# zaki699/Real-Time-Video-Quality-Analysis

Hardware: AMD Instinct MI355X
Metric: frames/sec (higher is better)
Workload: dtype u8->f32 (SSE/bins/SAD exact int); 1 GPU; 1920x1080 full suite (motion-SAD, DCT, temporal-DCT, Canny, ORB count, gray+colour hist) + PSNR/SSIM; id=c3, streams=1, inflight=2, collective=none, rehearsal_single_device=False, resident=HBM, ssim_mode=gauss, pixfmt=bgr24, dct_mode=block8, motion=sad, parallelism=1 stream/GPU x1, overlap=True, launched_by=direct

## Files before the change

### real-time-video-quality-analysis_amd/csrc/k_gray_hist.hip

```cpp
#include "vqa_dev.hpp"
#include "vqa_kernels.hpp"
#include "vqa_math.hpp"

namespace vqa {

enum { F_GRAY_HIST = 1, F_COLOR_HIST = 2, F_SUM2 = 4 };

__device__ __forceinline__ uint32_t byte_of(const uint32_t *d, int k) { return (d[k >> 2] >> ((k & 3) * 8)) & 0xffu; }

template <bool VEC>
__global__ __launch_bounds__(256) void k_bgr2gray_hist(const uint8_t *__restrict__ bgr, int h, int w,
                                                       int64_t frame_stride, int64_t row_stride,
                                                       uint8_t *__restrict__ gray, int gp, int64_t plane_stride,
                                                       vqa_frame_metrics *__restrict__ res, uint32_t flags)
{
    __shared__ uint32_t lh[4 * 256 * 8];
    __shared__ unsigned long long red[4];
    const int f = blockIdx.y;
    const bool hg = (flags & F_GRAY_HIST) && res, hc = (flags & F_COLOR_HIST) && res;
    const bool any_hist = hg || hc;
    if (any_hist) {
        for (int i = threadIdx.x; i < 4 * 256 * 8; i += 256) lh[i] = 0;
        __syncthreads();
    }
    const unsigned cp = threadIdx.x & 7u;
    const uint8_t *src = bgr + (int64_t)f * frame_stride;
    uint8_t *dst = gray + (int64_t)f * plane_stride;
    const int cpr = (w + 15) >> 4;
    const int total = h * cpr;
    unsigned long long s2 = 0;
    for (int c = blockIdx.x * 256 + threadIdx.x; c < total; c += gridDim.x * 256) {
        const int y = c / cpr;
        const int x0 = (c - y * cpr) << 4;
        const uint8_t *p = src + (int64_t)y * row_stride + (int64_t)x0 * 3;
        uint32_t d[12];
        int npx = 16;
        if (VEC) {
            const uint4 v0 = ((const uint4 *)p)[0], v1 = ((const uint4 *)p)[1], v2 = ((const uint4 *)p)[2];
            d[0] = v0.x; d[1] = v0.y; d[2] = v0.z; d[3] = v0.w;
            d[4] = v1.x; d[5] = v1.y; d[6] = v1.z; d[7] = v1.w;
            d[8] = v2.x; d[9] = v2.y; d[10] = v2.z; d[11] = v2.w;
        } else {
            npx = min(16, w - x0);
#pragma unroll
            for (int k = 0; k < 12; k++) d[k] = 0;
            for (int k = 0; k < npx * 3; k++) d[k >> 2] |= (uint32_t)p[k] << ((k & 3) * 8);
        }
        uint32_t g[16];
        uint32_t sq = 0;
#pragma unroll
        for (int i = 0; i < 16; i++) {
            const uint32_t b = byte_of(d, 3 * i), gg = byte_of(d, 3 * i + 1), r = byte_of(d, 3 * i + 2);
            g[i] = bgr2gray_u8(b, gg, r);
            if (VEC || i < npx) {
                sq += g[i] * g[i];
                if (hg) atomicAdd(&lh[(g[i] << 3) | cp], 1u);
                if (hc) {
                    atomicAdd(&lh[((256u + b) << 3) | cp], 1u);
                    atomicAdd(&lh[((512u + gg) << 3) | cp], 1u);
                    atomicAdd(&lh[((768u + r) << 3) | cp], 1u);
                }
            }
        }
        s2 += sq;
        uint8_t *q = dst + (int64_t)y * gp + x0;
        if (VEC) {
            uint4 o;
            o.x = g[0] | (g[1] << 8) | (g[2] << 16) | (g[3] << 24);
            o.y = g[4] | (g[5] << 8) | (g[6] << 16) | (g[7] << 24);
            o.z = g[8] | (g[9] << 8) | (g[10] << 16) | (g[11] << 24);
            o.w = g[12] | (g[13] << 8) | (g[14] << 16) | (g[15] << 24);
            *(uint4 *)q = o;
        } else {
            for (int i = 0; i < npx; i++) q[i] = (uint8_t)g[i];
        }
    }
    if (!res) return;
    if (any_hist) {
        __syncthreads();
        for (int i = threadIdx.x; i < 4 * 256; i += 256) {
            const uint4 c0 = *(const uint4 *)&lh[i * 8], c1 = *(const uint4 *)&lh[i * 8 + 4];
            const uint32_t v = c0.x + c0.y + c0.z + c0.w + c1.x + c1.y + c1.z + c1.w;
            if (v) {
                const int which = i >> 8, bin = i & 255;
                uint32_t *gdst = which == 0 ? &res[f].hist_gray[bin] : &res[f].hist_bgr[which - 1][bin];
                atomicAdd(gdst, v);
            }
        }
    }
    if (flags & F_SUM2) {
        const unsigned long long t = block_sum_u64(s2, red);
        if (threadIdx.x == 0 && t) atomicAdd((unsigned long long *)&res[f].sum_gray2, t);
    }
}

__global__ __launch_bounds__(256) void k_resize_planes(const uint8_t *__restrict__ bgr, int h, int w,
                                                       int64_t frame_stride, int64_t row_stride, int rw, int rh,
                                                       const int32_t *__restrict__ xofs, const int32_t *__restrict__ xa,
                                                       const int32_t *__restrict__ yofs, const int32_t *__restrict__ yb,
                                                       int mode, uint8_t *__restrict__ planeA,
                                                       uint8_t *__restrict__ planeB, int pp, int64_t plane_stride,
                                                       vqa_frame_metrics *__restrict__ res, uint32_t flags)
{
    __shared__ uint32_t lh[4][256];
    __shared__ unsigned long long red[4];
    const int f = blockIdx.y;
    const bool hg = (flags & F_GRAY_HIST) && res, hc = (flags & F_COLOR_HIST) && res;
    if (hg || hc) {
        for (int i = threadIdx.x; i < 4 * 256; i += 256) (&lh[0][0])[i] = 0;
        __syncthreads();
    }
    const int idx = blockIdx.x * 256 + threadIdx.x;
    unsigned long long s2 = 0;
    if (idx < rw * rh) {
        const int oy = idx / rw, ox = idx - oy * rw;
        int sx0, sx1, sy0, sy1, a0, a1, b0, b1;
        if (mode == 1) {
            sx0 = 2 * ox; sx1 = sx0 + 1; sy0 = 2 * oy; sy1 = sy0 + 1;
            a0 = a1 = b0 = b1 = 0;
        } else {
            sx0 = xofs[ox]; sx1 = min(sx0 + 1, w - 1);
            a0 = xa[2 * ox]; a1 = xa[2 * ox + 1];
            const int sy = yofs[oy];
            sy0 = min(max(sy, 0), h - 1); sy1 = min(max(sy + 1, 0), h - 1);
            b0 = yb[2 * oy]; b1 = yb[2 * oy + 1];
        }
        const uint8_t *src = bgr + (int64_t)f * frame_stride;
        const uint8_t *p00 = src + (int64_t)sy0 * row_stride + (int64_t)sx0 * 3;
        const uint8_t *p01 = src + (int64_t)sy0 * row_stride + (int64_t)sx1 * 3;
        const uint8_t *p10 = src + (int64_t)sy1 * row_stride + (int64_t)sx0 * 3;
        const uint8_t *p11 = src + (int64_t)sy1 * row_stride + (int64_t)sx1 * 3;
        uint32_t c00[3], c01[3], c10[3], c11[3];
#pragma unroll
        for (int k = 0; k < 3; k++) { c00[k] = p00[k]; c01[k] = p01[k]; c10[k] = p10[k]; c11[k] = p11[k]; }
        const uint32_t g00 = bgr2gray_u8(c00[0], c00[1], c00[2]), g01 = bgr2gray_u8(c01[0], c01[1], c01[2]);
        const uint32_t g10 = bgr2gray_u8(c10[0], c10[1], c10[2]), g11 = bgr2gray_u8(c11[0], c11[1], c11[2]);
        uint32_t ga, rc[3];
        if (mode == 1) {
            ga = (g00 + g01 + g10 + g11 + 2) >> 2;
#pragma unroll
            for (int k = 0; k < 3; k++) rc[k] = (c00[k] + c01[k] + c10[k] + c11[k] + 2) >> 2;
        } else {
            ga = resize_vcombine((int)(g00 * a0 + g01 * a1), (int)(g10 * a0 + g11 * a1), b0, b1);
#pragma unroll
            for (int k = 0; k < 3; k++)
                rc[k] = resize_vcombine((int)(c00[k] * a0 + c01[k] * a1), (int)(c10[k] * a0 + c11[k] * a1), b0, b1);
        }
        const uint32_t gb = bgr2gray_u8(rc[0], rc[1], rc[2]);
        planeA[(int64_t)f * plane_stride + (int64_t)oy * pp + ox] = (uint8_t)ga;
        if (planeB) planeB[(int64_t)f * plane_stride + (int64_t)oy * pp + ox] = (uint8_t)gb;
        s2 = (unsigned long long)(ga * ga);
        if (hg) atomicAdd(&lh[0][gb], 1u);
        if (hc) { atomicAdd(&lh[1][rc[0]], 1u); atomicAdd(&lh[2][rc[1]], 1u); atomicAdd(&lh[3][rc[2]], 1u); }
    }
    if (!res) return;
    if (hg || hc) {
        __syncthreads();
        for (int i = threadIdx.x; i < 4 * 256; i += 256) {
            const uint32_t v = (&lh[0][0])[i];
            if (v) {
                const int which = i >> 8, bin = i & 255;
                atomicAdd(which == 0 ? &res[f].hist_gray[bin] : &res[f].hist_bgr[which - 1][bin], v);
            }
        }
    }
    if (flags & F_SUM2) {
        const unsigned long long t = block_sum_u64(s2, red);
        if (threadIdx.x == 0 && t) atomicAdd((unsigned long long *)&res[f].sum_gray2, t);
    }
}


void launch_bgr2gray_hist(hipStream_t st, const uint8_t *bgr, int n, int h, int w, int64_t frame_stride,
                          int64_t row_stride, uint8_t *gray, int gp, int64_t plane_stride, vqa_frame_metrics *res,
                          bool gray_hist, bool color_hist, bool sum2)
{
    if (n <= 0) return;
    const uint32_t flags = (gray_hist ? F_GRAY_HIST : 0) | (color_hist ? F_COLOR_HIST : 0) | (sum2 ? F_SUM2 : 0);
    const bool vec = (w % 16 == 0) && (((uintptr_t)bgr | (uintptr_t)gray) % 16 == 0) && (frame_stride % 16 == 0) &&
                     (row_stride % 16 == 0) && (gp % 16 == 0) && (plane_stride % 16 == 0);
    const int chunks = h * ((w + 15) / 16);
    int bpf = (chunks + 256 * 8 - 1) / (256 * 8);
    bpf = bpf < 1 ? 1 : (bpf > 256 ? 256 : bpf);
    dim3 grid(bpf, n), block(256);
    if (vec)
        hipLaunchKernelGGL(k_bgr2gray_hist<true>, grid, block, 0, st, bgr, h, w, frame_stride, row_stride, gray, gp,
                           plane_stride, res, flags);
    else
        hipLaunchKernelGGL(k_bgr2gray_hist<false>, grid, block, 0, st, bgr, h, w, frame_stride, row_stride, gray, gp,
                           plane_stride, res, flags);
}

void launch_resize_planes(hipStream_t st, const uint8_t *bgr, int n, int h, int w, int64_t frame_stride,
                          int64_t row_stride, int rw, int rh, const int32_t *xofs, const int32_t *xa,
                          const int32_t *yofs, const int32_t *yb, int mode, uint8_t *planeA, uint8_t *planeB, int pp,
                          int64_t plane_stride, vqa_frame_metrics *res, bool gray_hist, bool color_hist, bool sum2)
{
    if (n <= 0) return;
    const uint32_t flags = (gray_hist ? F_GRAY_HIST : 0) | (color_hist ? F_COLOR_HIST : 0) | (sum2 ? F_SUM2 : 0);
    dim3 grid((rw * rh + 255) / 256, n), block(256);
    hipLaunchKernelGGL(k_resize_planes, grid, block, 0, st, bgr, h, w, frame_stride, row_stride, rw, rh, xofs, xa, yofs,
                       yb, mode, planeA, planeB, pp, plane_stride, res, flags);
}

}
```

### real-time-video-quality-analysis_amd/csrc/vqa_capi.hip

```cpp
#include <hip/hip_runtime.h>

#include <cmath>
#include <cstddef>
#include <cstdio>
#include <cstdlib>
#include <cstring>
#include <map>
#include <string>
#include <tuple>
#include <vector>

#include "vqa_kernels.hpp"

using namespace vqa;

namespace {

struct dbuf {
    void *p = nullptr;
    size_t cap = 0;
};

struct hbuf {
    void *p = nullptr;
// ... 656 lines not shown

void vqa_default_params(vqa_params *p)
{
    if (!p) return;
    memset(p, 0, sizeof *p);
    p->canny_low = 100;
    p->canny_high = 200;
    p->sad_range = 7;
    p->dct_mode = VQA_DCT_AUTO;
}

int vqa_create(int device, vqa_ctx **out)
{
    if (!out) return VQA_ERR_INVALID;
    *out = nullptr;
    int n = 0;
    if (hipGetDeviceCount(&n) != hipSuccess || n <= 0) return VQA_ERR_NO_DEVICE;
    if (device < 0 || device >= n) return VQA_ERR_NO_DEVICE;
    vqa_ctx *c = new (std::nothrow) vqa_ctx();
    if (!c) return VQA_ERR_OOM;
    c->device = device;
    if (hipSetDevice(device) != hipSuccess || hipStreamCreateWithFlags(&c->stream, hipStreamNonBlocking) != hipSuccess) {
        delete c;
        return VQA_ERR_HIP;
    }
    c->dct_wave_slots = dct8_wave_slots();
    if (const char *e = getenv("VQA_OVERLAP")) c->opt_overlap = atoi(e) != 0;
#ifdef VQA_TEST_SEAMS
    if (const char *e = getenv("VQA_HYST_MAX_ROUNDS")) c->seam_hyst_max_rounds = atoi(e) > 0 ? atoi(e) : 0;
    if (const char *e = getenv("VQA_HYST_RESCUE_MAX_ROUNDS")) c->seam_hyst_rescue_max_rounds = atoi(e) > 0 ? atoi(e) : 0;
    if (const char *e = getenv("VQA_FAIL_ENSURE_AT")) c->seam_fail_at = atol(e);
    if (const char *e = getenv("VQA_FB_CHUNK_BYTES")) c->seam_fb_chunk_bytes = atoll(e);
#endif
    *out = c;
    return VQA_OK;
}

int vqa_set_option(vqa_ctx *c, int option, int value)
{
    if (!c) return VQA_ERR_INVALID;
    if (busy(c)) return VQA_ERR_STATE;
    switch (option) {
    case VQA_OPT_OVERLAP: c->opt_overlap = value != 0; return VQA_OK;
    case VQA_OPT_HYST_STATS: c->opt_hyst_stats = value != 0; return VQA_OK;
    default: return VQA_ERR_INVALID;
    }
}

int vqa_get_option(const vqa_ctx *c, int option, int *value)
{
    if (!c || !value) return VQA_ERR_INVALID;
    switch (option) {
    case VQA_OPT_OVERLAP: *value = c->opt_overlap ? 1 : 0; return VQA_OK;
    case VQA_OPT_HYST_STATS: *value = c->opt_hyst_stats ? 1 : 0; return VQA_OK;
    default: return VQA_ERR_INVALID;
    }
}

int vqa_build_flavour(void)
{
    int f = 0;
#ifdef VQA_AB_VARIANTS
    f |= 1;
#endif
#ifdef VQA_TEST_SEAMS
    f |= 2;
#endif
    return f;
}

static void release_scratch(vqa_ctx *c)
{
    dbuf *bufs[] = {&c->gray_full, &c->planeA, &c->planeB, &c->state, &c->res_dev, &c->partials, &c->tile_flags,
                    &c->dirty0, &c->dirty1, &c->again_dev, &c->stage_frames, &c->stage_prev, &c->dct_scratch,
                    &c->dct_pe, &c->dct_pt, &c->qres_dev, &c->qpartials, &c->qstage_ref, &c->qstage_dist,
                    &c->qms_pyr, &c->qms_dev, &c->vif_pyr, &c->vif_acc, &c->vif_dev, &c->adm_pyr, &c->adm_part, &c->adm_sums, &c->mot_acc, &c->mot_stage, &c->mot_prev, &c->fb_tmp, &c->fb_blur, &c->fb_img, &c->fb_R, &c->fb_M, &c->fb_flow0, &c->fb_flow1, &c->fb_part};
    for (dbuf *b : bufs) release(*b);
    for (auto &kv : c->tabs) free_table(kv.second.v);
    for (auto &kv : c->fb_tabs) free_table(kv.second.v);
    for (auto &kv : c->dct_mats) free_table(kv.second.v);
    for (auto &kv : c->fft_plans) free_table(kv.second.v);
    c->tabs.clear(); c->fb_tabs.clear(); c->dct_mats.clear(); c->fft_plans.clear();
    for (hbuf *b : {&c->res_host, &c->qres_host, &c->qms_host, &c->vif_host, &c->adm_host, &c->mot_host}) {
        if (b->p) (void)hipHostFree(b->p);
        b->p = nullptr; b->cap = 0;
    }
    c->last_n = 0; c->last_has_full = c->last_has_state = c->last_has_planes = false;
}

int vqa_trim(vqa_ctx *c)
{
    if (!c) return VQA_ERR_INVALID;
    if (busy(c)) return VQA_ERR_STATE;
    HIPCHK(c, hipSetDevice(c->device));
    if (int rc = sync_all(c)) return rc;
    prof_collect(c);
    release_scratch(c);
    (void)hipGetLastError();
    return VQA_OK;
}

int vqa_destroy(vqa_ctx *c)
{
    if (!c) return VQA_ERR_INVALID;
    (void)hipSetDevice(c->device);
    (void)sync_all(c);
    release_scratch(c);
    for (auto &t : c->ev_open) { (void)hipEventDestroy(std::get<1>(t)); (void)hipEventDestroy(std::get<2>(t)); }
    for (hipEvent_t e : c->ev_pool) (void)hipEventDestroy(e);
    for (int i = 0; i < 3; i++) {
        if (c->side[i]) (void)hipStreamDestroy(c->side[i]);
        if (c->ev_join[i]) (void)hipEventDestroy(c->ev_join[i]);
    }
    if (c->ev_fork) (void)hipEventDestroy(c->ev_fork);
    if (c->ev_xctx) (void)hipEventDestroy(c->ev_xctx);
    for (int i = 0; i < 6; i++)
        if (c->fb_ev[i]) (void)hipEventDestroy(c->fb_ev[i]);
    (void)hipStreamDestroy(c->stream);
    delete c;
    return VQA_OK;
}

const char *vqa_last_hip_error(const vqa_ctx *c) { return c ? c->last_err.c_str() : ""; }

int vqa_alloc_pinned(vqa_ctx *c, size_t bytes, void **out)
{
    if (!c || !out || !bytes) return VQA_ERR_INVALID;
    HIPCHK(c, hipSetDevice(c->device));
    HIPCHK(c, hipHostMalloc(out, bytes, hipHostMallocDefault));
    return VQA_OK;
}
int vqa_free_pinned(vqa_ctx *c, void *p)
{
    if (!c || !p) return VQA_ERR_INVALID;
    HIPCHK(c, hipHostFree(p));
    return VQA_OK;
}
static bool host_byte_is_pinned(const void *p)
{
    hipPointerAttribute_t a;
    memset(&a, 0, sizeof a);
    if (hipPointerGetAttributes(&a, p) != hipSuccess) {
        (void)hipGetLastError();
        return false;
    }
    return a.type == hipMemoryTypeHost;
}
int vqa_host_is_pinned(vqa_ctx *c, const void *p, size_t bytes, int *out)
{
    if (!c || !p || !out || !bytes) return VQA_ERR_INVALID;
    *out = (host_byte_is_pinned(p) && host_byte_is_pinned((const uint8_t *)p + (bytes - 1))) ? 1 : 0;
    return VQA_OK;
}
int vqa_alloc_device(vqa_ctx *c, size_t bytes, void **out)
{
    if (!c || !out || !bytes) return VQA_ERR_INVALID;
    HIPCHK(c, hipSetDevice(c->device));
    HIPCHK(c, hipMalloc(out, bytes));
    return VQA_OK;
}
int vqa_free_device(vqa_ctx *c, void *p)
{
    if (!c || !p) return VQA_ERR_INVALID;
    HIPCHK(c, hipFree(p));
    return VQA_OK;
}
int vqa_copy_h2d(vqa_ctx *c, void *dst, const void *src, size_t bytes)
{
    if (!c || !dst || !src) return VQA_ERR_INVALID;
    HIPCHK(c, hipSetDevice(c->device));
    HIPCHK(c, hipMemcpyAsync(dst, src, bytes, hipMemcpyHostToDevice, c->stream));
    return VQA_OK;
}
int vqa_stream_wait(vqa_ctx *waiter, vqa_ctx *signaler)
{
    if (!waiter || !signaler || waiter == signaler) return VQA_ERR_INVALID;
    if (waiter->device != signaler->device) return VQA_ERR_INVALID;
    HIPCHK(waiter, hipSetDevice(waiter->device));
    if (!signaler->ev_xctx) HIPCHK(waiter, hipEventCreateWithFlags(&signaler->ev_xctx, hipEventDisableTiming));
    HIPCHK(waiter, hipEventRecord(signaler->ev_xctx, signaler->stream));
    HIPCHK(waiter, hipStreamWaitEvent(waiter->stream, signaler->ev_xctx, 0));
    return VQA_OK;
}
int vqa_copy_d2h(vqa_ctx *c, void *dst, const void *src, size_t bytes)
{
    if (!c || !dst || !src) return VQA_ERR_INVALID;
    HIPCHK(c, hipSetDevice(c->device));
    HIPCHK(c, hipMemcpyAsync(dst, src, bytes, hipMemcpyDeviceToHost, c->stream));
    return VQA_OK;
}
int vqa_sync(vqa_ctx *c)
{
    if (!c) return VQA_ERR_INVALID;
    return sync_all(c);
}
void *vqa_stream(vqa_ctx *c) { return c ? (void *)c->stream : nullptr; }
extern "C" __attribute__((visibility("hidden"))) int vqa_ctx_device_(const vqa_ctx *c) { return c->device; }
extern "C" __attribute__((visibility("hidden"))) void *vqa_ctx_stream_(const vqa_ctx *c) { return (void *)c->stream; }

static int drain_failed_submit(vqa_ctx *c, int rc, bool touched)
{
    if (rc != VQA_OK && touched) {
        const std::string why = c->last_err;
        (void)sync_all(c);
        (void)hipGetLastError();
        prof_discard(c);
        c->last_err = why;
    }
    return rc;
}

static int complexity_submit_body(vqa_ctx *c, const uint8_t *frames, const uint8_t *prev0, int mem_kind, int n, int h, int w,
                                  int64_t frame_stride, int64_t row_stride, uint32_t mask, const vqa_params *params,
                                  bool &touched)
{
    if (!c || !frames || n <= 0 || h <= 0 || w <= 0) return VQA_ERR_INVALID;
    if (mem_kind != VQA_MEM_HOST && mem_kind != VQA_MEM_DEVICE) return VQA_ERR_INVALID;
    if (!mask || (mask & ~VQA_M_ALL)) return VQA_ERR_INVALID;
    if (row_stride < (int64_t)3 * w || frame_stride < row_stride * (h - 1) + (int64_t)3 * w) return VQA_ERR_INVALID;
    if (c->pend_c) return VQA_ERR_STATE;
    vqa_params P;
    if (params) P = *params; else vqa_default_params(&P);
    for (int i = 0; i < 9; i++)
        if (P.reserved[i]) return VQA_ERR_INVALID;
    if (P.motion_mode != VQA_MOTION_SAD && P.motion_mode != VQA_MOTION_FARNEBACK) return VQA_ERR_INVALID;
    if (P.sad_range < 0 || P.sad_range > 7) return VQA_ERR_INVALID;
    if (P.resize_w < 0 || P.resize_h < 0 || ((P.resize_w == 0) != (P.resize_h == 0))) return VQA_ERR_INVALID;
    if (P.dct_mode < VQA_DCT_AUTO || P.dct_mode > VQA_DCT_FULL) return VQA_ERR_INVALID;
    if ((int64_t)h * w > (1ll << 28)) return VQA_ERR_UNSUPPORTED;
    HIPCHK(c, hipSetDevice(c->device));
    hipStream_t st = c->stream;
    touched = true;

    const int rw = P.resize_w ? P.resize_w : w, rh = P.resize_h ? P.resize_h : h;
    const bool resized = !(rw == w && rh == h);
    const int ph = rh, pw = rw;
    const int pp = align_up(pw, 64), gp = align_up(w, 64);
    const bool want_gh = mask & VQA_M_GRAY_HIST, want_ch = mask & VQA_M_COLOR_HIST, want_dct = mask & VQA_M_DCT;
    const bool want_t = mask & VQA_M_TEMPORAL_DCT, want_e = mask & VQA_M_EDGE, want_m = mask & VQA_M_MOTION;
    const bool want_orb = mask & VQA_M_ORB;
    const bool batch_has_prev0 = prev0 != nullptr;

    const uint8_t *dframes = frames, *dprev = prev0;
    if (mem_kind == VQA_MEM_HOST) {
        const size_t rbytes = (size_t)3 * w, fbytes = rbytes * h;
        const bool padded = (size_t)row_stride != rbytes;
        int rc = ensure(c, c->stage_frames, fbytes * n);
        if (rc) return rc;
        if (!padded && (size_t)frame_stride == fbytes) {
            HIPCHK(c, hipMemcpyAsync(c->stage_frames.p, frames, fbytes * n, hipMemcpyHostToDevice, st));
        } else {
            for (int i = 0; i < n; i++) {
                uint8_t *dst = (uint8_t *)c->stage_frames.p + fbytes * i;
                const uint8_t *src = frames + (int64_t)i * frame_stride;
                if (padded)
                    HIPCHK(c, hipMemcpy2DAsync(dst, rbytes, src, (size_t)row_stride, rbytes, h, hipMemcpyHostToDevice, st));
                else
                    HIPCHK(c, hipMemcpyAsync(dst, src, fbytes, hipMemcpyHostToDevice, st));
            }
        }
        dframes = (const uint8_t *)c->stage_frames.p;
        if (batch_has_prev0) {
            rc = ensure(c, c->stage_prev, fbytes);
            if (rc) return rc;
            if (padded)
                HIPCHK(c, hipMemcpy2DAsync(c->stage_prev.p, rbytes, prev0, (size_t)row_stride, rbytes, h,
                                           hipMemcpyHostToDevice, st));
            else
                HIPCHK(c, hipMemcpyAsync(c->stage_prev.p, prev0, fbytes, hipMemcpyHostToDevice, st));
            dprev = (const uint8_t *)c->stage_prev.p;
        }
        frame_stride = (int64_t)fbytes;
        row_stride = (int64_t)rbytes;
    }

    int rc = ensure(c, c->res_dev, sizeof(vqa_frame_metrics) * (size_t)n);
    if (rc) return rc;
    rc = ensure_pinned(c, c->res_host, sizeof(vqa_frame_metrics) * (size_t)n);
    if (rc) return rc;
    HIPCHK(c, hipMemsetAsync(c->res_dev.p, 0, sizeof(vqa_frame_metrics) * (size_t)n, st));
    vqa_frame_metrics *const res_all = (vqa_frame_metrics *)c->res_dev.p;
    const uint8_t *const dframes_all = dframes, *const dprev_all = dprev;
    const int n_all = n;

    const int SLICE = 32768;
    auto run_slice = [&](const int a0) -> int {
    const int n = n_all - a0 < SLICE ? n_all - a0 : SLICE;
    const uint8_t *dframes = dframes_all + (int64_t)a0 * frame_stride;
    const uint8_t *dprev = a0 ? dframes_all + (int64_t)(a0 - 1) * frame_stride : dprev_all;
    const bool has_prev0 = a0 > 0 || batch_has_prev0;
    vqa_frame_metrics *res = res_all + a0;

    const bool want_plane = want_gh || want_ch || want_dct || want_t || want_e;
    const bool need_full = (!resized && want_plane) || want_m;
    const bool need_planes = resized && want_plane;
    const int64_t full_stride = (int64_t)h * gp, plane_stride = (int64_t)ph * pp;
    uint8_t *gfull = nullptr, *pA = nullptr, *pB = nullptr;
    if (need_full) {
        rc = ensure(c, c->gray_full, (size_t)full_stride * (n + 1));
        if (rc) return rc;
        gfull = (uint8_t *)c->gray_full.p;
        const bool prev_needed = has_prev0 && (want_m || (!resized && want_t));
        prof_scope ps_(c, VQA_K_GRAY_HIST);
        if (prev_needed)
            launch_bgr2gray_hist(st, dprev, 1, h, w, frame_stride, row_stride, gfull, gp, full_stride, nullptr, false,
                                 false, false);
        launch_bgr2gray_hist(st, dframes, n, h, w, frame_stride, row_stride, gfull + full_stride, gp, full_stride, res,
                             !resized && want_gh, !resized && want_ch, !resized && want_dct);
    }
    if (need_planes) {
        resize_tabs T;
        rc = get_tabs(c, h, w, rh, rw, T);
        if (rc) return rc;
        rc = ensure(c, c->planeA, (size_t)plane_stride * (n + 1));
        if (rc) return rc;
        rc = ensure(c, c->planeB, (size_t)plane_stride * n);
        if (rc) return rc;
        pA = (uint8_t *)c->planeA.p;
        pB = (uint8_t *)c->planeB.p;
        prof_scope ps_(c, VQA_K_RESIZE);
        if (has_prev0 && want_t)
            launch_resize_planes(st, dprev, 1, h, w, frame_stride, row_stride, rw, rh, T.xofs, T.xa, T.yofs, T.yb,
                                 T.mode, pA, nullptr, pp, plane_stride, nullptr, false, false, false);
        launch_resize_planes(st, dframes, n, h, w, frame_stride, row_stride, rw, rh, T.xofs, T.xa, T.yofs, T.yb, T.mode,
                             pA + plane_stride, pB, pp, plane_stride, res, want_gh, want_ch, want_dct);
    } else if (!resized) {
        pA = gfull;
        pB = gfull + full_stride;
    }

    int dct_mode_eff = P.dct_mode;
    if (dct_mode_eff == VQA_DCT_AUTO) dct_mode_eff = ((int64_t)ph * pw <= 128 * 128) ? VQA_DCT_FULL : VQA_DCT_BLOCK8;
    const bool use_side[3] = {c->opt_overlap && want_m && P.motion_mode == VQA_MOTION_SAD, c->opt_overlap && want_e,
                              c->opt_overlap && (want_dct || want_t) && dct_mode_eff == VQA_DCT_FULL && (want_m || want_e)};
    const bool overlap = use_side[0] || use_side[1] || use_side[2];
    hipStream_t st_sad = st, st_canny = st, st_dct = st;
    if (overlap) {
        for (int i = 0; i < 3; i++) {
            if (!use_side[i]) continue;
            if (!c->side[i]) HIPCHK(c, hipStreamCreateWithFlags(&c->side[i], hipStreamNonBlocking));
            if (!c->ev_join[i]) HIPCHK(c, hipEventCreateWithFlags(&c->ev_join[i], hipEventDisableTiming));
        }
        if (!c->ev_fork) HIPCHK(c, hipEventCreateWithFlags(&c->ev_fork, hipEventDisableTiming));
        HIPCHK(c, hipEventRecord(c->ev_fork, st));
        if (use_side[0]) { st_sad = c->side[0]; HIPCHK(c, hipStreamWaitEvent(st_sad, c->ev_fork, 0)); }
        if (use_side[1]) { st_canny = c->side[1]; HIPCHK(c, hipStreamWaitEvent(st_canny, c->ev_fork, 0)); }
        if (use_side[2]) { st_dct = c->side[2]; HIPCHK(c, hipStreamWaitEvent(st_dct, c->ev_fork, 0)); }
    }

    if (want_dct || want_t) {
        const int mode = dct_mode_eff;
        if (mode == VQA_DCT_BLOCK8) {
            const int pb = dct8_blocks_per_frame(ph, pw);
            rc = ensure(c, c->partials, sizeof(double) * 2 * (size_t)pb * n);
            if (rc) return rc;
            prof_scope ps_(c, VQA_K_DCT8);
            launch_dct8(st, pA, pp, plane_stride, n, ph, pw, want_dct, want_t, has_prev0, (double *)c->partials.p, res, c->dct_wave_slots);
        } else {
            if (dct_fft_supported(ph, pw)) {
                dct_fft_plan Pw, Ph;
                rc = get_fft_plan(c, pw, &Pw);
                if (rc) return rc;
                rc = get_fft_plan(c, ph, &Ph);
                if (rc) return rc;
                const size_t tiles = (size_t)dct_fft_tiles(ph, pw);
                rc = ensure(c, c->dct_scratch, sizeof(float) * 2 * (size_t)ph * pw * n);
                if (rc) return rc;
                rc = ensure(c, c->dct_pe, sizeof(double) * tiles * n);
                if (rc) return rc;
                rc = ensure(c, c->dct_pt, sizeof(double) * tiles * n);
                if (rc) return rc;
                prof_scope ps_(c, VQA_K_DCT_FULL, st_dct);
                launch_dct_full_fft(st_dct, pA, pp, plane_stride, n, ph, pw, Pw, Ph, (float *)c->dct_scratch.p, (double *)c->dct_pe.p,
                                    (double *)c->dct_pt.p, want_dct, want_t, has_prev0, res);
            } else {
                float *cw = nullptr, *ch = nullptr;
                rc = get_dct_matrix(c, pw, &cw);
                if (rc) return rc;
                rc = get_dct_matrix(c, ph, &ch);
                if (rc) return rc;
                const size_t tiles = (size_t)((ph + 15) / 16) * ((pw + 15) / 16);
                rc = ensure(c, c->dct_scratch, sizeof(float) * (size_t)ph * pw * n);
                if (rc) return rc;
                rc = ensure(c, c->dct_pe, sizeof(double) * tiles * n);
                if (rc) return rc;
                rc = ensure(c, c->dct_pt, sizeof(double) * tiles * n);
                if (rc) return rc;
                prof_scope ps_(c, VQA_K_DCT_FULL, st_dct);
                launch_dct_full(st_dct, pA, pp, plane_stride, n, ph, pw, cw, ch, (float *)c->dct_scratch.p,
                                (double *)c->dct_pe.p, (double *)c->dct_pt.p, want_dct, want_t, has_prev0, res);
            }
        }
    }

    if (want_m && P.motion_mode == VQA_MOTION_SAD) {
        prof_scope ps_(c, VQA_K_SAD, st_sad);
        launch_block_sad(st_sad, gfull, gp, full_stride, n, h, w, P.sad_range, has_prev0, res);
    } else if (want_m) {
        prof_scope ps_(c, VQA_K_FARNEBACK);
        rc = run_farneback(c, st, gfull, gp, full_stride, n, h, w, has_prev0, res);
        if (rc) return rc;
    }

    c->last_has_state = false;
    if (want_e) {
        const int ww = (pw + 63) / 64;
        const size_t words = (size_t)n * ((ph + 63) / 64) * ww * 64;
        const unsigned ntiles = canny_hyst_tiles(n, ph, pw);
        rc = ensure(c, c->state, sizeof(uint64_t) * words * 2);
        if (rc) return rc;
        rc = ensure(c, c->tile_flags, sizeof(uint32_t) * ntiles * 2);
        if (rc) return rc;
        const size_t NS = CANNY_HYST_SEGMENTS;
        rc = ensure(c, c->dirty0, sizeof(uint32_t) * ntiles * NS);
        if (rc) return rc;
        rc = ensure(c, c->dirty1, sizeof(uint32_t) * ntiles * NS);
        if (rc) return rc;
        rc = ensure(c, c->again_dev, sizeof(uint32_t) * 3 * n * NS);
        if (rc) return rc;
        unsigned long long *strong = (unsigned long long *)c->state.p, *weak = strong + words;
        unsigned *queued[2] = {(unsigned *)c->tile_flags.p, (unsigned *)c->tile_flags.p + ntiles};
        unsigned *lists[2] = {(unsigned *)c->dirty0.p, (unsigned *)c->dirty1.p};
        unsigned *counts = (unsigned *)c->again_dev.p;
        HIPCHK(c, hipMemsetAsync(queued[0], 0, sizeof(uint32_t) * ntiles * 2, st_canny));
        HIPCHK(c, hipMemsetAsync(counts, 0, sizeof(uint32_t) * 3 * n * NS, st_canny));
        auto cnt = [&](int r) { return counts + (size_t)(r % 3) * n * NS; };
        int lo = P.canny_low, hi = P.canny_high;
        if (lo > hi) { int t = lo; lo = hi; hi = t; }
        {
            prof_scope ps_(c, VQA_K_CANNY_NMS, st_canny);
            launch_canny_nms(st_canny, pB, pp, plane_stride, n, ph, pw, lo, hi, strong, weak, res);
        }
        int round = 0;
        {
            prof_scope ps_(c, VQA_K_CANNY_HYST, st_canny);
            launch_canny_hyst_all(st_canny, strong, weak, n, ph, pw, queued[1], lists[1], cnt(1), res, c->opt_hyst_stats);
        }
        {
            prof_scope ps_(c, VQA_K_CANNY_HYST, st_canny);
            const canny_geom cg = canny_tiles(ph, pw);
            int WIDE = (cg.tiles_x * cg.tiles_y > 1024 && n < 256) ? 8 : 6;
#ifdef VQA_AB_VARIANTS
            { static const int e = ab_knob("VQA_HYST_WIDE", 0); if (e > 0) WIDE = e; }
#endif
            for (round = 1; round <= WIDE; round++) {
                const int in = round & 1, out = in ^ 1;
#ifdef VQA_AB_VARIANTS
                static const bool trace = ab_knob("VQA_HYST_TRACE", 0) != 0;
                if (trace) {
                    std::vector<uint32_t> hc((size_t)n * NS);
                    (void)hipStreamSynchronize(st_canny);
                    (void)hipMemcpy(hc.data(), cnt(round), sizeof(uint32_t) * hc.size(), hipMemcpyDeviceToHost);
                    unsigned long long tot = 0;
                    for (uint32_t v : hc) tot += v;
                    fprintf(stderr, "[hyst] round %d: %llu of %u tiles queued\n", round, tot, ntiles);
                }
#endif
                launch_canny_hyst_list(st_canny, strong, weak, n, ph, pw, queued[in], lists[in], cnt(round), queued[out], lists[out],
                                       cnt(round + 1), cnt(round + 2), res, c->opt_hyst_stats);
            }
            unsigned *tc[2];
            tc[round & 1] = cnt(round);
            tc[(round & 1) ^ 1] = cnt(round + 1);
            launch_canny_hyst_tail(st_canny, strong, weak, n, ph, pw, lists[0], tc[0], queued[0], lists[1], tc[1], queued[1],
                                   round & 1, res, c->opt_hyst_stats, c->seam_hyst_max_rounds, c->seam_hyst_rescue_max_rounds);
        }
        launch_canny_finish(st_canny, strong, n, ph, pw, res);
        c->last_has_state = true;
    }

    if (want_orb) {
        resize_tabs T64;
        rc = get_tabs(c, h, w, 64, 64, T64);
        if (rc) return rc;
        prof_scope ps_(c, VQA_K_ORB);
        launch_orb64(st, dframes, n, h, w, frame_stride, row_stride, T64.xofs, T64.xa, T64.yofs, T64.yb, T64.mode, res);
    }
    if (overlap) {
        hipStream_t ss[3] = {st_sad, st_canny, st_dct};
        for (int i = 0; i < 3; i++) {
            if (!use_side[i]) continue;
            HIPCHK(c, hipEventRecord(c->ev_join[i], ss[i]));
            HIPCHK(c, hipStreamWaitEvent(st, c->ev_join[i], 0));
        }
    }
    c->last_n = n; c->last_has_full = need_full; c->last_has_planes = need_planes;
    return VQA_OK;
    };
    for (int a0 = 0; a0 < n_all; a0 += SLICE)
        if (const int src = run_slice(a0)) return src;
    const bool has_prev0 = batch_has_prev0;

    HIPCHK(c, hipGetLastError());
    if (want_gh || want_ch) {
        HIPCHK(c, hipMemcpyAsync(c->res_host.p, c->res_dev.p, sizeof(vqa_frame_metrics) * (size_t)n, hipMemcpyDeviceToHost, st));
        c->pend_c_tail_only = false;
    } else {
        const size_t off = offsetof(vqa_frame_metrics, sum_gray2), tail = sizeof(vqa_frame_metrics) - off;
        HIPCHK(c, hipMemcpy2DAsync((uint8_t *)c->res_host.p + off, sizeof(vqa_frame_metrics), (uint8_t *)c->res_dev.p + off,
                                   sizeof(vqa_frame_metrics), tail, (size_t)n, hipMemcpyDeviceToHost, st));
        c->pend_c_tail_only = true;
    }
    c->pend_c = n;
    c->pend_c_prev0 = has_prev0;
    c->last_h = h; c->last_w = w; c->last_ph = ph; c->last_pw = pw; c->last_pp = pp; c->last_gp = gp;
    c->last_resized = resized;
    return VQA_OK;
}

int vqa_complexity_submit(vqa_ctx *c, const uint8_t *frames, const uint8_t *prev0, int mem_kind, int n, int h, int w,
                          int64_t frame_stride, int64_t row_stride, uint32_t mask, const vqa_params *params)
{
    bool touched = false;
    const int rc = complexity_submit_body(c, frames, prev0, mem_kind, n, h, w, frame_stride, row_stride, mask, params, touched);
    return drain_failed_submit(c, rc, touched);
}

int vqa_complexity_wait(vqa_ctx *c, vqa_frame_metrics *out, int n)
{
    if (!c || !out) return VQA_ERR_INVALID;
    if (!c->pend_c || n != c->pend_c) return VQA_ERR_STATE;
    HIPCHK(c, hipStreamSynchronize(c->stream));
    prof_collect(c);
    memcpy(out, c->res_host.p, sizeof(vqa_frame_metrics) * (size_t)n);
    for (int i = 0; i < n; i++) {
        if (c->pend_c_tail_only) memset(&out[i], 0, offsetof(vqa_frame_metrics, sum_gray2));
        out[i].has_prev = (i > 0 || c->pend_c_prev0) ? 1u : 0u;
    }
    c->pend_c = 0;
    for (int i = 0; i < n; i++)
        if (out[i].hyst_overflow == 1u) {
            c->last_err = "Canny hysteresis of frame " + std::to_string(i) + " of " + std::to_string(n) +
                          " stopped before its fixpoint (edge_count " + std::to_string(out[i].edge_count) +
                          " would be a lower bound): records withheld";
            memset(out, 0, sizeof(vqa_frame_metrics) * (size_t)n);
            return VQA_ERR_INCOMPLETE;
        }
    return VQA_OK;
}

extern "C++" {

static bool bad_batch_args(const vqa_ctx *c, const void *ref, const void *dist, int mem_kind, int n, const vqa_plane_desc *planes,
                           int n_planes)
{
    return !c || !ref || !dist || n <= 0 || !planes || n_planes <= 0 || n_planes > 4 ||
           (mem_kind != VQA_MEM_HOST && mem_kind != VQA_MEM_DEVICE);
}

struct plane_batch {
    int depth, bps;
    int64_t span;
};

template <class F> static int check_planes(const vqa_plane_desc *planes, int n_planes, plane_batch &B, F limits)
{
    B.depth = planes[0].bit_depth == 0 ? 8 : planes[0].bit_depth;
    if (B.depth < 8 || B.depth > 16) return VQA_ERR_INVALID;
    B.bps = B.depth > 8 ? 2 : 1;
    B.span = 0;
    for (int p = 0; p < n_planes; p++) {
        const vqa_plane_desc &d = planes[p];
        if ((d.bit_depth == 0 ? 8 : d.bit_depth) != B.depth) return VQA_ERR_INVALID;
        if (B.bps == 2 && ((d.offset | d.row_stride | (int64_t)d.pixel_step) & 1)) return VQA_ERR_INVALID;
        if (d.width <= 0 || d.height <= 0 || d.offset < 0 || d.pixel_step <= 0 ||
            d.row_stride < (int64_t)d.width * d.pixel_step - (d.pixel_step - B.bps))
            return VQA_ERR_INVALID;
        if (int rc = limits(d)) return rc;
        const int64_t end = d.offset + (int64_t)(d.height - 1) * d.row_stride + (int64_t)(d.width - 1) * d.pixel_step + B.bps;
        B.span = end > B.span ? end : B.span;
    }
    return VQA_OK;
}

static int side_and_area_limits(const vqa_plane_desc &d, int min_dim)
{
    if (d.width < min_dim || d.height < min_dim) return VQA_ERR_UNSUPPORTED;
    if ((int64_t)d.width * d.height > (1ll << 28)) return VQA_ERR_UNSUPPORTED;
    return VQA_OK;
}

static int stage(vqa_ctx *c, dbuf &buf, const uint8_t *&frames, size_t bytes)
{
    if (int rc = ensure(c, buf, bytes)) return rc;
    HIPCHK(c, hipMemcpyAsync(buf.p, frames, bytes, hipMemcpyHostToDevice, c->stream));
    frames = (const uint8_t *)buf.p;
    return VQA_OK;
}

static int stage_pair(vqa_ctx *c, int mem_kind, int n, int64_t span, const uint8_t *&ref, int64_t ref_fs, const uint8_t *&dist,
                      int64_t dist_fs)
{
    if (mem_kind != VQA_MEM_HOST) return VQA_OK;
    if (int rc = stage(c, c->qstage_ref, ref, (size_t)(n - 1) * ref_fs + span)) return rc;
    return stage(c, c->qstage_dist, dist, (size_t)(n - 1) * dist_fs + span);
}

constexpr int QSLICE = 32768;

template <class F> static void for_each_slice(int n, F body)
{
    for (int a0 = 0; a0 < n; a0 += QSLICE) body(a0, n - a0 < QSLICE ? n - a0 : QSLICE);
}

template <class F> static void for_each_group(const vqa_plane_desc *planes, int n_planes, F body)
{
    bool done[4] = {false, false, false, false};
    for (int p = 0; p < n_planes; p++) {
        if (done[p]) continue;
        int idx[4], cnt = 0;
        for (int q = p; q < n_planes; q++) {
// ... 412 lines not shown
```

### real-time-video-quality-analysis_amd/csrc/vqa_kernels.hpp

```cpp
#pragma once
#include <hip/hip_runtime.h>
#include <stdint.h>

#include "../../include/vqa.h"

#ifdef VQA_AB_VARIANTS
#include <cstdlib>
#endif

namespace vqa {

inline int ab_knob(const char *name, int dflt)
{
#ifdef VQA_AB_VARIANTS
    const char *e = getenv(name);
    return e ? atoi(e) : dflt;
#else
    (void)name;
    return dflt;
#endif
}

void launch_bgr2gray_hist(hipStream_t st, const uint8_t *bgr, int n, int h, int w, int64_t frame_stride,
                          int64_t row_stride, uint8_t *gray, int gp, int64_t plane_stride, vqa_frame_metrics *res,
                          bool gray_hist, bool color_hist, bool sum2);
void launch_resize_planes(hipStream_t st, const uint8_t *bgr, int n, int h, int w, int64_t frame_stride,
                          int64_t row_stride, int rw, int rh, const int32_t *xofs, const int32_t *xa,
                          const int32_t *yofs, const int32_t *yb, int mode, uint8_t *planeA, uint8_t *planeB, int pp,
                          int64_t plane_stride, vqa_frame_metrics *res, bool gray_hist, bool color_hist, bool sum2);

void launch_orb64(hipStream_t st, const uint8_t *bgr, int n, int h, int w, int64_t frame_stride, int64_t row_stride,
                  const int32_t *xofs, const int32_t *xa, const int32_t *yofs, const int32_t *yb, int mode,
                  vqa_frame_metrics *res);

int dct8_blocks_per_frame(int h, int w);
int dct8_wave_slots();
void launch_dct8(hipStream_t st, const uint8_t *planes, int pitch, int64_t plane_stride, int n, int h, int w,
                 bool energy, bool temporal, bool first_has_prev, double *partials, vqa_frame_metrics *res, int wave_slots);

void launch_dct_full(hipStream_t st, const uint8_t *planes, int pitch, int64_t plane_stride, int n, int h, int w,
                     const float *cw, const float *ch, float *scratch, double *pe, double *pt, bool energy,
                     bool temporal, bool first_has_prev, vqa_frame_metrics *res);

void launch_dct_full_finalize(hipStream_t st, const double *pe, const double *pt, int tiles, int n, vqa_frame_metrics *res,
                              bool energy, bool temporal, bool first_has_prev);

constexpr int DCT_FFT_MAX_PASSES = 12;
struct dct_fft_plan {
    int n, npass;
    int radix[DCT_FFT_MAX_PASSES];
    int m[DCT_FFT_MAX_PASSES], tstep[DCT_FFT_MAX_PASSES];
    uint32_t ns_magic[DCT_FFT_MAX_PASSES];
    const float2 *tw;
    const float2 *post;
};
bool dct_fft_factor(int n, int radix[DCT_FFT_MAX_PASSES], int *npass);
bool dct_fft_supported(int h, int w);
int dct_fft_tiles(int h, int w);
void launch_dct_full_fft(hipStream_t st, const uint8_t *planes, int pitch, int64_t plane_stride, int n, int h, int w,
                         const dct_fft_plan &plan_w, const dct_fft_plan &plan_h, float *scratch, double *pe, double *pt,
                         bool energy, bool temporal, bool first_has_prev, vqa_frame_metrics *res);

struct canny_geom {
    int tiles_x, tiles_y;
};
canny_geom canny_tiles(int h, int w);
void launch_canny_nms(hipStream_t st, const uint8_t *gray, int pitch, int64_t plane_stride, int n, int h, int w,
                      int low, int high, unsigned long long *strong, unsigned long long *weak,
                      vqa_frame_metrics *res);
unsigned canny_hyst_tiles(int n, int h, int w);
constexpr int CANNY_HYST_SEGMENTS = 16;
void launch_canny_hyst_all(hipStream_t st, unsigned long long *strong, const unsigned long long *weak, int n, int h,
                           int w, unsigned *queued, unsigned *out_list, unsigned *out_count, vqa_frame_metrics *res,
                           int stats);
void launch_canny_hyst_list(hipStream_t st, unsigned long long *strong, const unsigned long long *weak, int n, int h,
                            int w, unsigned *in_queued, const unsigned *in_list, const unsigned *in_count,
                            unsigned *out_queued, unsigned *out_list, unsigned *out_count, unsigned *zero_count,
                            vqa_frame_metrics *res, int stats);
void launch_canny_hyst_tail(hipStream_t st, unsigned long long *strong, const unsigned long long *weak, int n, int h,
                            int w, unsigned *list0, unsigned *cnt0, unsigned *q0, unsigned *list1, unsigned *cnt1,
                            unsigned *q1, int first_in, vqa_frame_metrics *res, int stats, int max_rounds, int rescue_max_rounds);
constexpr int CANNY_HYST_MAX_ROUNDS = 1 << 16;
void launch_canny_finish(hipStream_t st, const unsigned long long *strong, int n, int h, int w, vqa_frame_metrics *res);

void launch_block_sad(hipStream_t st, const uint8_t *planes, int pitch, int64_t plane_stride, int n, int h, int w,
                      int range, bool first_has_prev, vqa_frame_metrics *res);

struct fb_taps {
    float k[32];
    int ksize;
};
struct fb_poly {
    float g[11], xg[11], xxg[11];
    double ig11, ig03, ig33, ig55;
};
struct fb_resize_tabs {
    int32_t *xofs = nullptr, *yofs = nullptr;
    float *xa = nullptr, *yb = nullptr;
    int mode = 0;
    int32_t *cols = nullptr, *rows = nullptr;
    int nc = 0, nr = 0;
    int32_t *sx = nullptr, *sy = nullptr;
    int span_x32 = 0, span_y8 = 0, span_y32 = 0;
};
void launch_fb_blur(hipStream_t st, const uint8_t *gray, int pitch, int64_t plane_stride, int planes, int h, int w,
                    const fb_taps &T, const int32_t *cols, int nc, const int32_t *rows, int nr, float *tmp, float *out);
bool launch_fb_level(hipStream_t st, const uint8_t *gray, int pitch, int64_t plane_stride, int planes, int h, int w,
                     const fb_taps &K, const fb_resize_tabs *T, float *out, int lh, int lw);
void launch_fb_resize(hipStream_t st, const float *src, int sh, int sw, int cn, float *dst, int dh, int dw, int images,
                      const fb_resize_tabs &T, float mul, bool apply_mul);
void launch_fb_polyexp(hipStream_t st, const float *in, int planes, int h, int w, const fb_poly &C, float *out);
void launch_fb_iter(hipStream_t st, const float *R, const float *flow, int pairs, int h, int w, float *flow_out,
                    double *mag_partials = nullptr);
int fb_iter_blocks(int pairs, int h, int w);
int fb_iter_max_blocks(int h, int w);
void launch_fb_mag_finalize(hipStream_t st, const double *partials, int nblk, int pairs, int h, int w, bool first_valid,
                            vqa_frame_metrics *res);
#ifdef VQA_AB_VARIANTS
void launch_fb_update(hipStream_t st, const float *R, const float *flow, int pairs, int h, int w, float *M);
void launch_fb_update_first(hipStream_t st, const float *R, const float *coarse, int ch, int cw, const fb_resize_tabs &T,
                            float mul, int pairs, int h, int w, float *M);
void launch_fb_blur_solve(hipStream_t st, const float *M, int pairs, int h, int w, float *flow);
#endif
#ifdef VQA_AB_VARIANTS
int fb_mag_blocks();
void launch_fb_mag(hipStream_t st, const float *flow, int pairs, int h, int w, double *partials, bool first_valid,
                   vqa_frame_metrics *res);
#endif

inline void group_slots(const vqa_plane_desc *planes, const int *idx, int count, int64_t offset[4], int plane_index[4])
{
    for (int i = 0; i < 4; i++) {
        const int p = idx[i < count ? i : 0];
        if (offset) offset[i] = planes[p].offset;
        if (plane_index) plane_index[i] = p;
    }
}

int ssim_gauss_blocks(int h, int w);
void launch_quality_gauss(hipStream_t st, const uint8_t *ref, const uint8_t *dist, int n, int64_t ref_frame_stride,
                          int64_t dist_frame_stride, const vqa_plane_desc *planes, const int *idx, int count,
                          int n_planes, double *partials, int64_t partial_plane_stride, vqa_plane_metrics *res, int depth);
void launch_quality_ffmpeg(hipStream_t st, const uint8_t *ref, const uint8_t *dist, int n, int64_t ref_frame_stride,
                           int64_t dist_frame_stride, const vqa_plane_desc *planes, const int *idx, int count,
                           int n_planes, double *partials, int64_t partial_plane_stride, vqa_plane_metrics *res, int depth);
int ssim_ffmpeg_blocks(int h, int w);

constexpr int MS_LEVELS = 5;
constexpr int MS_MIN_DIM = 161;
struct ms_layout {
    int w[MS_LEVELS], h[MS_LEVELS];
    int64_t off[MS_LEVELS];
    int64_t total;
};
inline ms_layout ms_levels(int n, int count, int h, int w)
{
    ms_layout L;
    L.w[0] = w; L.h[0] = h; L.off[0] = 0;
    int64_t at = 0;
    for (int s = 1; s < MS_LEVELS; s++) {
        L.w[s] = (L.w[s - 1] + 1) / 2;
        L.h[s] = (L.h[s - 1] + 1) / 2;
        L.off[s] = at;
        at += 2 * (int64_t)n * count * L.h[s] * L.w[s];
    }
    L.total = at;
    return L;
}
void launch_ms_pyramid(hipStream_t st, const uint8_t *ref, const uint8_t *dist, int n, int64_t ref_frame_stride,
                       int64_t dist_frame_stride, const vqa_plane_desc *planes, const int *idx, int count, int depth,
                       float *scratch);
void launch_quality_ms_level(hipStream_t st, const uint8_t *ref, const uint8_t *dist, int n, int64_t ref_frame_stride,
                             int64_t dist_frame_stride, const vqa_plane_desc *planes, const int *idx, int count, int n_planes,
                             double *partials, int64_t partial_plane_stride, vqa_plane_metrics *res, int depth, int level,
                             const float *scratch, vqa_ms_scales *ms);
void launch_ms_finalize(hipStream_t st, const double *partials, int64_t cs_offset, int bpp, int n, double count,
                        int plane_index, int n_planes, int level, vqa_ms_scales *ms);
void launch_ms_combine(hipStream_t st, const vqa_ms_scales *ms, int n_entries, vqa_plane_metrics *res);

constexpr int VIF_LEVELS = 4;
constexpr int VIF_MIN_DIM = 16;
struct vif_layout {
    int w[VIF_LEVELS], h[VIF_LEVELS];
    int64_t off[VIF_LEVELS];
    int64_t total;
};
inline vif_layout vif_levels(int n, int count, int h, int w)
{
    vif_layout L;
    L.w[0] = w; L.h[0] = h; L.off[0] = 0;
    int64_t at = 0;
    for (int s = 1; s < VIF_LEVELS; s++) {
        L.w[s] = L.w[s - 1] / 2;
        L.h[s] = L.h[s - 1] / 2;
        L.off[s] = at;
        at += 2 * (int64_t)n * count * L.h[s] * L.w[s];
    }
    L.total = at;
    return L;
}
void launch_vif_decimate(hipStream_t st, const uint8_t *ref, const uint8_t *dist, int n, int64_t ref_frame_stride,
                         int64_t dist_frame_stride, const vqa_plane_desc *planes, const int *idx, int count, int depth,
                         int level, float *scratch);
void launch_vif_stats(hipStream_t st, const uint8_t *ref, const uint8_t *dist, int n, int64_t ref_frame_stride,
                      int64_t dist_frame_stride, const vqa_plane_desc *planes, const int *idx, int count, int n_planes,
                      int depth, int level, const float *scratch, long long *acc);
void launch_vif_finalize(hipStream_t st, const long long *acc, int n_entries, vqa_vif_metrics *res);

constexpr int ADM_LEVELS = 4;
constexpr int ADM_MIN_DIM = 16;
struct adm_layout {
    int w[ADM_LEVELS + 1], h[ADM_LEVELS + 1];
    int64_t off[ADM_LEVELS];
    int64_t total;
};
inline adm_layout adm_levels(int n, int count, int h, int w)
{
    adm_layout L;
    L.w[0] = w; L.h[0] = h; L.off[0] = 0;
    int64_t at = 0;
    for (int s = 1; s <= ADM_LEVELS; s++) {
        L.w[s] = (L.w[s - 1] + 1) / 2;
        L.h[s] = (L.h[s - 1] + 1) / 2;
        if (s < ADM_LEVELS) {
            L.off[s] = at;
            at += 2 * (int64_t)n * count * L.h[s] * L.w[s];
        }
    }
    L.total = at;
    return L;
}
inline int adm_tiles(int bh, int bw) { return ((bw + 31) / 32) * ((bh + 15) / 16); }
struct adm_region { int top, bottom, left, right; int64_t area; };
inline adm_region adm_region_of(int bh, int bw)
{
    adm_region r;
    r.left = (int)(bw * 0.1 - 0.5);
    r.top = (int)(bh * 0.1 - 0.5);
    r.right = bw - r.left;
    r.bottom = bh - r.top;
    r.area = (int64_t)(r.bottom - r.top) * (r.right - r.left);
    return r;
}
void adm_rf(int scale, double *rf_hv, double *rf_d);
void launch_adm_scale(hipStream_t st, const uint8_t *ref, const uint8_t *dist, int n, int64_t ref_frame_stride,
                      int64_t dist_frame_stride, const vqa_plane_desc *planes, const int *idx, int count, int depth, int scale,
                      float *scratch, double *part);
void launch_adm_reduce(hipStream_t st, const double *part, int n, const vqa_plane_desc *planes, const int *idx, int count,
                       int n_planes, int scale, double *sums);
void adm_finalize(const double *sums, int h, int w, vqa_adm_metrics *out);

constexpr int MOTION_MIN_DIM = 16;
constexpr int MOTION_RADIUS = 2;
constexpr double MOTION_TAPS[5] = {0.054488685, 0.244201342, 0.402619947, 0.244201342, 0.054488685};
void launch_motion_sad(hipStream_t st, const uint8_t *ref, const uint8_t *prev0, int n, int64_t frame_stride,
                       const vqa_plane_desc *planes, const int *idx, int count, int n_planes, int depth, long long *acc);

}
```

Measured before the change: 37410 frames/s.

## Merge prev-frame gray conversion into main launch, widen blocks and histogram copies

Folds the separate single-frame launch that converts the previous frame to gray into the main batched launch by adding an extra grid row, which removes one kernel launch per call. Blocks grow from 256 to 1024 threads, and the shared histogram gets 16 privatized copies per bin instead of 8 to cut atomic contention. The final reduction over copies is rotated to avoid bank conflicts, and the sum reduction reuses the histogram shared buffer. The cost is 64KB of shared memory per block, which can limit occupancy, and fewer blocks per frame.

```diff
diff --git a/real-time-video-quality-analysis_amd/csrc/k_gray_hist.hip b/real-time-video-quality-analysis_amd/csrc/k_gray_hist.hip
--- a/real-time-video-quality-analysis_amd/csrc/k_gray_hist.hip
+++ b/real-time-video-quality-analysis_amd/csrc/k_gray_hist.hip
@@ -8,28 +8,33 @@
 
 __device__ __forceinline__ uint32_t byte_of(const uint32_t *d, int k) { return (d[k >> 2] >> ((k & 3) * 8)) & 0xffu; }
 
+constexpr int GH_COPIES = 16, GH_LOG2C = 4, GH_THREADS = 1024;
+static_assert((1 << GH_LOG2C) == GH_COPIES, "the copy index is the low GH_LOG2C bits of an entry's address");
+
 template <bool VEC>
-__global__ __launch_bounds__(256) void k_bgr2gray_hist(const uint8_t *__restrict__ bgr, int h, int w,
-                                                       int64_t frame_stride, int64_t row_stride,
-                                                       uint8_t *__restrict__ gray, int gp, int64_t plane_stride,
-                                                       vqa_frame_metrics *__restrict__ res, uint32_t flags)
-{
-    __shared__ uint32_t lh[4 * 256 * 8];
-    __shared__ unsigned long long red[4];
-    const int f = blockIdx.y;
+__global__ __launch_bounds__(GH_THREADS) void k_bgr2gray_hist(const uint8_t *__restrict__ bgr,
+                                                              const uint8_t *__restrict__ prev0, int h, int w,
+                                                              int64_t frame_stride, int64_t row_stride,
+                                                              uint8_t *__restrict__ gray, int gp, int64_t plane_stride,
+                                                              vqa_frame_metrics *__restrict__ res, uint32_t flags)
+{
+    __shared__ uint32_t lh[4 * 256 * GH_COPIES];
+    const bool is_prev = prev0 && blockIdx.y == 0;
+    const int f = (int)blockIdx.y - (prev0 ? 1 : 0);
+    if (is_prev) res = nullptr;
     const bool hg = (flags & F_GRAY_HIST) && res, hc = (flags & F_COLOR_HIST) && res;
     const bool any_hist = hg || hc;
     if (any_hist) {
-        for (int i = threadIdx.x; i < 4 * 256 * 8; i += 256) lh[i] = 0;
-        __syncthreads();
-    }
-    const unsigned cp = threadIdx.x & 7u;
-    const uint8_t *src = bgr + (int64_t)f * frame_stride;
+        for (int i = threadIdx.x; i < 256 * GH_COPIES; i += GH_THREADS) ((uint4 *)lh)[i] = make_uint4(0, 0, 0, 0);
+        __syncthreads();
+    }
+    const unsigned cp = threadIdx.x & (unsigned)(GH_COPIES - 1);
+    const uint8_t *src = is_prev ? prev0 : bgr + (int64_t)f * frame_stride;
     uint8_t *dst = gray + (int64_t)f * plane_stride;
     const int cpr = (w + 15) >> 4;
     const int total = h * cpr;
     unsigned long long s2 = 0;
-    for (int c = blockIdx.x * 256 + threadIdx.x; c < total; c += gridDim.x * 256) {
+    for (int c = blockIdx.x * GH_THREADS + threadIdx.x; c < total; c += gridDim.x * GH_THREADS) {
         const int y = c / cpr;
         const int x0 = (c - y * cpr) << 4;
         const uint8_t *p = src + (int64_t)y * row_stride + (int64_t)x0 * 3;
@@ -54,11 +59,11 @@
             g[i] = bgr2gray_u8(b, gg, r);
             if (VEC || i < npx) {
                 sq += g[i] * g[i];
-                if (hg) atomicAdd(&lh[(g[i] << 3) | cp], 1u);
+                if (hg) atomicAdd(&lh[(g[i] << GH_LOG2C) | cp], 1u);
                 if (hc) {
-                    atomicAdd(&lh[((256u + b) << 3) | cp], 1u);
-                    atomicAdd(&lh[((512u + gg) << 3) | cp], 1u);
-                    atomicAdd(&lh[((768u + r) << 3) | cp], 1u);
+                    atomicAdd(&lh[((256u + b) << GH_LOG2C) | cp], 1u);
+                    atomicAdd(&lh[((512u + gg) << GH_LOG2C) | cp], 1u);
+                    atomicAdd(&lh[((768u + r) << GH_LOG2C) | cp], 1u);
                 }
             }
         }
@@ -78,9 +83,10 @@
     if (!res) return;
     if (any_hist) {
         __syncthreads();
-        for (int i = threadIdx.x; i < 4 * 256; i += 256) {
-            const uint4 c0 = *(const uint4 *)&lh[i * 8], c1 = *(const uint4 *)&lh[i * 8 + 4];
-            const uint32_t v = c0.x + c0.y + c0.z + c0.w + c1.x + c1.y + c1.z + c1.w;
+        for (int i = threadIdx.x; i < 4 * 256; i += GH_THREADS) {
+            uint32_t v = 0;
+#pragma unroll
+            for (int k = 0; k < GH_COPIES; k++) v += lh[(i << GH_LOG2C) | ((k + i) & (GH_COPIES - 1))];
             if (v) {
                 const int which = i >> 8, bin = i & 255;
                 uint32_t *gdst = which == 0 ? &res[f].hist_gray[bin] : &res[f].hist_bgr[which - 1][bin];
@@ -89,7 +95,7 @@
         }
     }
     if (flags & F_SUM2) {
-        const unsigned long long t = block_sum_u64(s2, red);
+        const unsigned long long t = block_sum_u64(s2, (unsigned long long *)lh);
         if (threadIdx.x == 0 && t) atomicAdd((unsigned long long *)&res[f].sum_gray2, t);
     }
 }
@@ -171,24 +177,24 @@
 }
 
 
-void launch_bgr2gray_hist(hipStream_t st, const uint8_t *bgr, int n, int h, int w, int64_t frame_stride,
-                          int64_t row_stride, uint8_t *gray, int gp, int64_t plane_stride, vqa_frame_metrics *res,
-                          bool gray_hist, bool color_hist, bool sum2)
+void launch_bgr2gray_hist(hipStream_t st, const uint8_t *bgr, const uint8_t *prev0, int n, int h, int w,
+                          int64_t frame_stride, int64_t row_stride, uint8_t *gray, int gp, int64_t plane_stride,
+                          vqa_frame_metrics *res, bool gray_hist, bool color_hist, bool sum2)
 {
     if (n <= 0) return;
     const uint32_t flags = (gray_hist ? F_GRAY_HIST : 0) | (color_hist ? F_COLOR_HIST : 0) | (sum2 ? F_SUM2 : 0);
-    const bool vec = (w % 16 == 0) && (((uintptr_t)bgr | (uintptr_t)gray) % 16 == 0) && (frame_stride % 16 == 0) &&
-                     (row_stride % 16 == 0) && (gp % 16 == 0) && (plane_stride % 16 == 0);
+    const bool vec = (w % 16 == 0) && (((uintptr_t)bgr | (uintptr_t)prev0 | (uintptr_t)gray) % 16 == 0) &&
+                     (frame_stride % 16 == 0) && (row_stride % 16 == 0) && (gp % 16 == 0) && (plane_stride % 16 == 0);
     const int chunks = h * ((w + 15) / 16);
-    int bpf = (chunks + 256 * 8 - 1) / (256 * 8);
+    int bpf = (chunks + GH_THREADS * 8 - 1) / (GH_THREADS * 8);
     bpf = bpf < 1 ? 1 : (bpf > 256 ? 256 : bpf);
-    dim3 grid(bpf, n), block(256);
+    dim3 grid(bpf, n + (prev0 ? 1 : 0)), block(GH_THREADS);
     if (vec)
-        hipLaunchKernelGGL(k_bgr2gray_hist<true>, grid, block, 0, st, bgr, h, w, frame_stride, row_stride, gray, gp,
-                           plane_stride, res, flags);
+        hipLaunchKernelGGL(k_bgr2gray_hist<true>, grid, block, 0, st, bgr, prev0, h, w, frame_stride, row_stride, gray,
+                           gp, plane_stride, res, flags);
     else
-        hipLaunchKernelGGL(k_bgr2gray_hist<false>, grid, block, 0, st, bgr, h, w, frame_stride, row_stride, gray, gp,
-                           plane_stride, res, flags);
+        hipLaunchKernelGGL(k_bgr2gray_hist<false>, grid, block, 0, st, bgr, prev0, h, w, frame_stride, row_stride, gray,
+                           gp, plane_stride, res, flags);
 }
 
 void launch_resize_planes(hipStream_t st, const uint8_t *bgr, int n, int h, int w, int64_t frame_stride,
diff --git a/real-time-video-quality-analysis_amd/csrc/vqa_capi.hip b/real-time-video-quality-analysis_amd/csrc/vqa_capi.hip
--- a/real-time-video-quality-analysis_amd/csrc/vqa_capi.hip
+++ b/real-time-video-quality-analysis_amd/csrc/vqa_capi.hip
@@ -982,11 +982,9 @@
         gfull = (uint8_t *)c->gray_full.p;
         const bool prev_needed = has_prev0 && (want_m || (!resized && want_t));
         prof_scope ps_(c, VQA_K_GRAY_HIST);
-        if (prev_needed)
-            launch_bgr2gray_hist(st, dprev, 1, h, w, frame_stride, row_stride, gfull, gp, full_stride, nullptr, false,
-                                 false, false);
-        launch_bgr2gray_hist(st, dframes, n, h, w, frame_stride, row_stride, gfull + full_stride, gp, full_stride, res,
-                             !resized && want_gh, !resized && want_ch, !resized && want_dct);
+        launch_bgr2gray_hist(st, dframes, prev_needed ? dprev : nullptr, n, h, w, frame_stride, row_stride,
+                             gfull + full_stride, gp, full_stride, res, !resized && want_gh, !resized && want_ch,
+                             !resized && want_dct);
     }
     if (need_planes) {
         resize_tabs T;
diff --git a/real-time-video-quality-analysis_amd/csrc/vqa_kernels.hpp b/real-time-video-quality-analysis_amd/csrc/vqa_kernels.hpp
--- a/real-time-video-quality-analysis_amd/csrc/vqa_kernels.hpp
+++ b/real-time-video-quality-analysis_amd/csrc/vqa_kernels.hpp
@@ -21,9 +21,9 @@
 #endif
 }
 
-void launch_bgr2gray_hist(hipStream_t st, const uint8_t *bgr, int n, int h, int w, int64_t frame_stride,
-                          int64_t row_stride, uint8_t *gray, int gp, int64_t plane_stride, vqa_frame_metrics *res,
-                          bool gray_hist, bool color_hist, bool sum2);
+void launch_bgr2gray_hist(hipStream_t st, const uint8_t *bgr, const uint8_t *prev0, int n, int h, int w,
+                          int64_t frame_stride, int64_t row_stride, uint8_t *gray, int gp, int64_t plane_stride,
+                          vqa_frame_metrics *res, bool gray_hist, bool color_hist, bool sum2);
 void launch_resize_planes(hipStream_t st, const uint8_t *bgr, int n, int h, int w, int64_t frame_stride,
                           int64_t row_stride, int rw, int rh, const int32_t *xofs, const int32_t *xa,
                           const int32_t *yofs, const int32_t *yb, int mode, uint8_t *planeA, uint8_t *planeB, int pp,
```

Measured after the change: 37690 frames/s, median of 6. Within noise of the previous version (+0.7%).
